# XiaRho/CMDA

Measured on AMD Instinct MI355X. Metric: training images/sec (512x512 image+event, MiT-B5), higher is better.
Workload: dtype bf16

## Files before the change

cmda_amd/csrc/attention.hip:

```cpp
#include "attention_common.h"

namespace {

struct AttnParams {
  const bf16_t* q;
  const bf16_t* kv;
  bf16_t* o;
  int B, N, Nk, heads, C;
  float scale;
  int q_per_block;
};

static inline int fwd_queries_per_block(int B, int N, int heads, bool full = false) {
  return (long)((N + 127) / 128) * heads * B < (full ? 512 : 1024) ? 64 : 128;
}

template <int MAXK, bool FULL = false>
__global__ __launch_bounds__(256, MAXK <= 256 ? 2 : 1) void attn_fwd_kernel(AttnParams p) {
  constexpr int NT = MAXK / 16;
  const int Nk = FULL ? MAXK : p.Nk;
  __shared__ __attribute__((aligned(1024))) bf16_t sK[MAXK * kHD];
  __shared__ __attribute__((aligned(1024))) bf16_t sV[MAXK * kHD];
  const int tid = threadIdx.x, lane = tid & 63, wid = tid >> 6, g = lane >> 4, l15 = lane & 15;
  const unsigned nqb = (unsigned)((p.N + p.q_per_block - 1) / p.q_per_block);
  const unsigned lb = xcd_logical_block(), bh = lb / nqb;
  const long qblk = lb - bh * nqb;
  const int h = (int)(bh % (unsigned)p.heads), b = (int)(bh / (unsigned)p.heads);
  const bf16_t* kbase = p.kv + (long)b * Nk * 2 * p.C + h * kHD;
  load_kv_tile<MAXK>(kbase, 2 * p.C, Nk, sK, wid, lane, 4);
  load_kv_tile<MAXK>(kbase + p.C, 2 * p.C, Nk, sV, wid, lane, 4);
  __syncthreads();
  const int nt = (Nk + 15) >> 4;
  const bf16_t* qb = p.q + (long)b * p.N * p.C + h * kHD;
  bf16_t* ob = p.o + (long)b * p.N * p.C + h * kHD;
  for (int pass = 0; pass < p.q_per_block / 64; ++pass) {
    const long q0 = qblk * p.q_per_block + pass * 64 + wid * 16;
    if (q0 >= p.N) break;
    u16x8 qf[2];
    load_qfrag(qb, q0, p.N, p.C, g, l15, qf);
    f32x4 pr[NT];
    float inv = 1.f;
    if constexpr (FULL) inv = scores_exp_full<NT>(sK, qf, p.scale, g, l15, pr);
    else scores_softmax<NT>(sK, qf, nt, Nk, p.scale, g, l15, pr);
    f32x4 oacc[4];
#pragma unroll
    for (int dt = 0; dt < 4; ++dt) oacc[dt] = f32x4{0.f, 0.f, 0.f, 0.f};
#pragma unroll
    for (int u = 0; u < NT / 2; ++u) {
      if (FULL || 2 * u < nt) {
        const u16x8 pb = pack_pair(pr[2 * u], pr[2 * u + 1]);
#pragma unroll
        for (int dt = 0; dt < 4; ++dt)
          oacc[dt] = mfma_bf16_16x16x32(frag_cols(sV, 32 * u + 4 * g, 32 * u + 16 + 4 * g, dt, l15), pb, oacc[dt]);
      }
    }
    if (q0 + l15 < p.N) {
#pragma unroll
      for (int dt = 0; dt < 4; ++dt) {
        if constexpr (FULL) oacc[dt] *= inv;
        const float v[4] = {oacc[dt][0], oacc[dt][1], oacc[dt][2], oacc[dt][3]};
        st4(ob + (q0 + l15) * p.C + 16 * dt + 4 * g, v);
      }
    }
  }
}

struct AttnBwdParams {
  const bf16_t* q;
  const bf16_t* kv;
  const bf16_t* d_o;
  bf16_t* dq;
  float* dkv32;
  bf16_t* dkv16;
  float* stats;
  int B, N, Nk, heads, C, q_per_block;
  float scale;
  int fwd_q_per_block;
  int spans;
};

template <bool FULL = false>
__global__ __launch_bounds__(256, 2) void attn_bwd_dq_kernel(AttnBwdParams p) {
  __shared__ __attribute__((aligned(1024))) bf16_t sK[kMaxK * kHD];
  __shared__ __attribute__((aligned(1024))) bf16_t sV[kMaxK * kHD];
  const int Nk = FULL ? kMaxK : p.Nk;
  const int tid = threadIdx.x, lane = tid & 63, wid = tid >> 6, g = lane >> 4, l15 = lane & 15;
  const unsigned nqb = (unsigned)((p.N + p.fwd_q_per_block - 1) / p.fwd_q_per_block);
  const unsigned lb = xcd_logical_block(), bh = lb / nqb;
  const long qblk = lb - bh * nqb;
  const int h = (int)(bh % (unsigned)p.heads), b = (int)(bh / (unsigned)p.heads);
  const bf16_t* kbase = p.kv + (long)b * Nk * 2 * p.C + h * kHD;
  load_kv_tile(kbase, 2 * p.C, Nk, sK, wid, lane, 4);
  load_kv_tile(kbase + p.C, 2 * p.C, Nk, sV, wid, lane, 4);
  __syncthreads();
  const int nt = (Nk + 15) >> 4;
  const long rowb = (long)b * p.N;
  const bf16_t* qb = p.q + rowb * p.C + h * kHD;
  const bf16_t* dob = p.d_o + rowb * p.C + h * kHD;
  bf16_t* dqb = p.dq + rowb * p.C + h * kHD;
  float* st = p.stats + ((long)b * p.heads + h) * p.N * 2;
  for (int pass = 0; pass < p.fwd_q_per_block / 64; ++pass) {
    const long q0 = qblk * p.fwd_q_per_block + pass * 64 + wid * 16;
    if (q0 >= p.N) break;
    u16x8 qf[2], dof[2];
    load_qfrag(qb, q0, p.N, p.C, g, l15, qf);
    load_qfrag(dob, q0, p.N, p.C, g, l15, dof);
    f32x4 pr[kNT], dp[kNT];
    float lse, inv = 1.f;
    if constexpr (FULL) inv = scores_exp_full(sK, qf, p.scale, g, l15, pr, &lse);
    else scores_softmax(sK, qf, nt, Nk, p.scale, g, l15, pr, &lse);
    float dsum = 0.f;
#pragma unroll
    for (int t = 0; t < kNT; ++t) {
      dp[t] = f32x4{0.f, 0.f, 0.f, 0.f};
      if (FULL || t < nt) {
#pragma unroll
        for (int kk = 0; kk < 2; ++kk) dp[t] = mfma_bf16_16x16x32(frag_rows(sV, 16 * t, kk, g, l15), dof[kk], dp[t]);
      }
#pragma unroll
      for (int r = 0; r < 4; ++r) dsum += pr[t][r] * dp[t][r];
    }
    dsum = col_sum(dsum);
    if constexpr (FULL) dsum *= inv;
#pragma unroll
    for (int t = 0; t < kNT; ++t)
#pragma unroll
      for (int r = 0; r < 4; ++r) {
        if constexpr (FULL) dp[t][r] = pr[t][r] * (dp[t][r] - dsum);
        else dp[t][r] = p.scale * pr[t][r] * (dp[t][r] - dsum);
      }
    f32x4 dqacc[4];
#pragma unroll
    for (int dt = 0; dt < 4; ++dt) dqacc[dt] = f32x4{0.f, 0.f, 0.f, 0.f};
#pragma unroll
    for (int u = 0; u < kNT / 2; ++u) {
      if (FULL || 2 * u < nt) {
        const u16x8 db = pack_pair(dp[2 * u], dp[2 * u + 1]);
#pragma unroll
        for (int dt = 0; dt < 4; ++dt)
          dqacc[dt] = mfma_bf16_16x16x32(frag_cols(sK, 32 * u + 4 * g, 32 * u + 16 + 4 * g, dt, l15), db, dqacc[dt]);
      }
    }
    if (q0 + l15 < p.N) {
#pragma unroll
      for (int dt = 0; dt < 4; ++dt) {
        if constexpr (FULL) dqacc[dt] *= p.scale * inv;
        const float v[4] = {dqacc[dt][0], dqacc[dt][1], dqacc[dt][2], dqacc[dt][3]};
        st4(dqb + (q0 + l15) * p.C + 16 * dt + 4 * g, v);
      }
      if (g == 0) {
        st[(q0 + l15) * 2 + 0] = lse;
        st[(q0 + l15) * 2 + 1] = dsum;
      }
    }
  }
}

constexpr int kRedPitch = 68;

template <int NW>
__global__ __launch_bounds__(64 * NW, NW == 4 ? 2 : 1) void attn_bwd_dkv_kernel(AttnBwdParams p) {
  __shared__ __attribute__((aligned(1024))) bf16_t sK[kKS * kHD];
  __shared__ __attribute__((aligned(1024))) bf16_t sV[kKS * kHD];
  constexpr int kStageBytes = NW * 2 * 32 * kHD * 2;
  constexpr int kRedBytes = 2 * kKS * kRedPitch * 4;
  __shared__ __attribute__((aligned(1024))) char sbuf[kStageBytes > kRedBytes ? kStageBytes : kRedBytes];
  const int tid = threadIdx.x, lane = tid & 63, wid = tid >> 6, g = lane >> 4, l15 = lane & 15;
  const unsigned lb = xcd_logical_block();
  const int ks = (int)(lb & 3);
  const unsigned span = (lb >> 2) % (unsigned)p.spans, bh = (lb >> 2) / (unsigned)p.spans;
  const int h = (int)(bh % (unsigned)p.heads), b = (int)(bh / (unsigned)p.heads);
  const int key0 = ks * kKS;
  if (key0 >= p.Nk) return;
  const int nkeys = min(kKS, p.Nk - key0);
  const bf16_t* kbase = p.kv + ((long)b * p.Nk + key0) * 2 * p.C + h * kHD;
  for (int i = wid; i < kKS / 8; i += NW) {
    const int row = 8 * i + (lane >> 3);
    const int chunk = (lane & 7) ^ (row & 7);
    const void* zero = static_cast<const void*>(g_attn_zero16);
    const bf16_t* src = kbase + (long)row * 2 * p.C + chunk * 8;
    glds16(row < nkeys ? static_cast<const void*>(src) : zero, reinterpret_cast<char*>(sK) + i * 1024);
    glds16(row < nkeys ? static_cast<const void*>(src + p.C) : zero, reinterpret_cast<char*>(sV) + i * 1024);
  }
  __syncthreads();
  const long rowb = (long)b * p.N;
  const bf16_t* qb = p.q + rowb * p.C + h * kHD;
  const bf16_t* dob = p.d_o + rowb * p.C + h * kHD;
  const float* st = p.stats + ((long)b * p.heads + h) * p.N * 2;
  bf16_t* sQw = reinterpret_cast<bf16_t*>(sbuf) + wid * 2 * 32 * kHD;
  bf16_t* sDOw = sQw + 32 * kHD;

  f32x4 dvacc[4][4], dkacc[4][4];
#pragma unroll
  for (int dt = 0; dt < 4; ++dt)
#pragma unroll
    for (int kt = 0; kt < 4; ++kt) dvacc[dt][kt] = dkacc[dt][kt] = f32x4{0.f, 0.f, 0.f, 0.f};

  const long qbeg = (long)span * p.q_per_block;
  const long qend = min((long)p.N, qbeg + p.q_per_block);
  for (long q32 = qbeg + 32 * wid; q32 < qend; q32 += 32 * NW) {
#pragma unroll
    for (int i = 0; i < 4; ++i) {
      const int row = 8 * i + (lane >> 3);
      const int chunk = (lane & 7) ^ (row & 7);
      const bool ok = q32 + row < p.N;
      const void* zero = static_cast<const void*>(g_attn_zero16);
      glds16(ok ? static_cast<const void*>(qb + (q32 + row) * p.C + chunk * 8) : zero, reinterpret_cast<char*>(sQw) + i * 1024);
      glds16(ok ? static_cast<const void*>(dob + (q32 + row) * p.C + chunk * 8) : zero, reinterpret_cast<char*>(sDOw) + i * 1024);
    }
    float lse[2][4], dd[2][4];
#pragma unroll
    for (int qt = 0; qt < 2; ++qt)
#pragma unroll
      for (int r = 0; r < 4; ++r) {
        const long qi = q32 + 16 * qt + 4 * g + r;
        const bool ok = qi < p.N;
        lse[qt][r] = ok ? st[qi * 2] : INFINITY;
        dd[qt][r] = ok ? st[qi * 2 + 1] : 0.f;
      }
    dma_wait<0>();
    f32x4 pr[2][4], ds[2][4];
#pragma unroll
    for (int qt = 0; qt < 2; ++qt) {
      u16x8 fq[2], fdo[2];
#pragma unroll
      for (int kk = 0; kk < 2; ++kk) {
        fq[kk] = frag_rows(sQw, 16 * qt, kk, g, l15);
        fdo[kk] = frag_rows(sDOw, 16 * qt, kk, g, l15);
      }
#pragma unroll
      for (int kt = 0; kt < 4; ++kt) {
        f32x4 s = f32x4{0.f, 0.f, 0.f, 0.f}, d = f32x4{0.f, 0.f, 0.f, 0.f};
#pragma unroll
        for (int kk = 0; kk < 2; ++kk) {
          s = mfma_bf16_16x16x32(fq[kk], frag_rows(sK, 16 * kt, kk, g, l15), s);
          d = mfma_bf16_16x16x32(fdo[kk], frag_rows(sV, 16 * kt, kk, g, l15), d);
        }
        const bool live = 16 * kt + l15 < nkeys;
#pragma unroll
        for (int r = 0; r < 4; ++r) {
          const float pv = live ? __expf(s[r] * p.scale - lse[qt][r]) : 0.f;
          pr[qt][kt][r] = pv;
          ds[qt][kt][r] = p.scale * pv * (d[r] - dd[qt][r]);
        }
      }
    }
#pragma unroll
    for (int dt = 0; dt < 4; ++dt) {
      const u16x8 fdoT = frag_cols(sDOw, 4 * g, 16 + 4 * g, dt, l15);
      const u16x8 fqT = frag_cols(sQw, 4 * g, 16 + 4 * g, dt, l15);
#pragma unroll
      for (int kt = 0; kt < 4; ++kt) {
        dvacc[dt][kt] = mfma_bf16_16x16x32(fdoT, pack_pair(pr[0][kt], pr[1][kt]), dvacc[dt][kt]);
        dkacc[dt][kt] = mfma_bf16_16x16x32(fqT, pack_pair(ds[0][kt], ds[1][kt]), dkacc[dt][kt]);
      }
    }
  }
  __syncthreads();
  float* red = reinterpret_cast<float*>(sbuf);
  for (int w = 0; w < NW; ++w) {
    if (wid == w) {
#pragma unroll
      for (int dt = 0; dt < 4; ++dt)
#pragma unroll
        for (int kt = 0; kt < 4; ++kt) {
          float* rk = red + (16 * kt + l15) * kRedPitch + 16 * dt + 4 * g;
          float* rv = rk + kKS * kRedPitch;
#pragma unroll
          for (int r = 0; r < 4; ++r) {
            rk[r] = (w ? rk[r] : 0.f) + dkacc[dt][kt][r];
            rv[r] = (w ? rv[r] : 0.f) + dvacc[dt][kt][r];
          }
        }
    }
    __syncthreads();
  }
  if (p.dkv16) {
    bf16_t* ob = p.dkv16 + ((long)b * p.Nk + key0) * 2 * p.C + h * kHD;
    for (int e = tid; e < kKS * kHD; e += 64 * NW) {
      const int kl = e >> 6, d = e & 63;
      if (kl < nkeys) {
        stf(ob + (long)kl * 2 * p.C + d, red[kl * kRedPitch + d]);
        stf(ob + (long)kl * 2 * p.C + p.C + d, red[(kKS + kl) * kRedPitch + d]);
      }
    }
    return;
  }
  float* ob = p.dkv32 + ((long)b * p.Nk + key0) * 2 * p.C + h * kHD;
  for (int e = tid; e < kKS * kHD; e += 64 * NW) {
    const int kl = e >> 6, d = e & 63;
    if (kl < nkeys) {
      atomicAdd(ob + (long)kl * 2 * p.C + d, red[kl * kRedPitch + d]);
      atomicAdd(ob + (long)kl * 2 * p.C + p.C + d, red[(kKS + kl) * kRedPitch + d]);
    }
  }
}


struct AttnX3Params {
  const float* q;
  const bf16_t* kvh;
  const bf16_t* kvl;
  float* o;
  int B, N, Nk, heads, C;
  float scale;
  int q_per_block;
};

static __device__ __forceinline__ void split4(const float (&x)[4], u16x4& hi, u16x4& lo) {
#pragma unroll
  for (int e = 0; e < 4; ++e) {
    const bf16_t h = f2bf(x[e]);
    hi[e] = h;
    lo[e] = f2bf(x[e] - bf2f(h));
  }
}

#ifndef CMDA_EMU
static __device__ __forceinline__ void wave_lds_sync() { asm volatile("s_waitcnt lgkmcnt(0)" ::: "memory"); }
#else
static inline void wave_lds_sync() { emu::wave_barrier(); }
#endif

static __device__ __forceinline__ void load_split_tile(const float* __restrict__ src, long ld, int nvalid, int rows, bf16_t* hi, bf16_t* lo,
                                                       int t, int nthr) {
  for (int i = t; i < rows * 16; i += nthr) {
    const int row = i >> 4, c4 = i & 15;
    float x[4] = {0.f, 0.f, 0.f, 0.f};
    if (row < nvalid) ld4(src + (long)row * ld + 4 * c4, x);
    u16x4 h, l;
    split4(x, h, l);
    const int off = row * kHD + ((((c4 >> 1) ^ (row & 7))) << 3) + ((c4 & 1) << 2);
    *reinterpret_cast<u16x4*>(hi + off) = h;
    *reinterpret_cast<u16x4*>(lo + off) = l;
  }
}

static __device__ __forceinline__ void load_qfrag_x3(const float* __restrict__ base, long row0, long nrows, int ld, int g, int l15,
                                                     u16x8 (&fh)[2], u16x8 (&fl)[2]) {
  long row = row0 + l15;
  if (row >= nrows) row = nrows - 1;
#pragma unroll
  for (int kk = 0; kk < 2; ++kk) {
    float a[4], b[4];
    ld4(base + row * ld + 32 * kk + 8 * g, a);
    ld4(base + row * ld + 32 * kk + 8 * g + 4, b);
    u16x4 ah, al, bh, bl;
    split4(a, ah, al);
    split4(b, bh, bl);
    fh[kk] = u16x8{ah[0], ah[1], ah[2], ah[3], bh[0], bh[1], bh[2], bh[3]};
    fl[kk] = u16x8{al[0], al[1], al[2], al[3], bl[0], bl[1], bl[2], bl[3]};
  }
}

static __device__ __forceinline__ f32x4 mfma_x3(u16x8 ah, u16x8 al, u16x8 bh, u16x8 bl, f32x4 c) {
  c = mfma_bf16_16x16x32(al, bh, c);
  c = mfma_bf16_16x16x32(ah, bl, c);
  return mfma_bf16_16x16x32(ah, bh, c);
}

static __device__ __forceinline__ void pack_pair_x3(const f32x4& a, const f32x4& b, u16x8& hi, u16x8& lo) {
#pragma unroll
  for (int r = 0; r < 4; ++r) {
    const bf16_t ha = f2bf(a[r]), hb = f2bf(b[r]);
    hi[r] = ha; hi[4 + r] = hb;
    lo[r] = f2bf(a[r] - bf2f(ha)); lo[4 + r] = f2bf(b[r] - bf2f(hb));
  }
}

static __device__ __forceinline__ void scores_softmax_x3(const bf16_t* sKh, const bf16_t* sKl, const u16x8 (&qh)[2], const u16x8 (&ql)[2],
                                                         int nt, int Nk, float scale, int g, int l15, f32x4 (&p)[kNT], float* lse_out = nullptr) {
#pragma unroll
  for (int t = 0; t < kNT; ++t) {
    p[t] = f32x4{0.f, 0.f, 0.f, 0.f};
    if (t < nt) {
#pragma unroll
      for (int kk = 0; kk < 2; ++kk)
// ... 242 lines not shown
        fdh[kk] = frag_rows(sDh, 16 * qt, kk, g, l15);
        fdl[kk] = frag_rows(sDl, 16 * qt, kk, g, l15);
      }
#pragma unroll
      for (int kt = 0; kt < 4; ++kt) {
        f32x4 s = f32x4{0.f, 0.f, 0.f, 0.f}, d = f32x4{0.f, 0.f, 0.f, 0.f};
#pragma unroll
        for (int kk = 0; kk < 2; ++kk) {
          s = mfma_x3(fqh[kk], fql[kk], frag_rows(sKh, 16 * kt, kk, g, l15), frag_rows(sKl, 16 * kt, kk, g, l15), s);
          d = mfma_x3(fdh[kk], fdl[kk], frag_rows(sVh, 16 * kt, kk, g, l15), frag_rows(sVl, 16 * kt, kk, g, l15), d);
        }
        const bool live = 16 * kt + l15 < nkeys;
#pragma unroll
        for (int r = 0; r < 4; ++r) {
          const float pv = live ? __expf(s[r] * p.scale - lse[qt][r]) : 0.f;
          pr[qt][kt][r] = pv;
          ds[qt][kt][r] = p.scale * pv * (d[r] - dd[qt][r]);
        }
      }
    }
#pragma unroll
    for (int dt = 0; dt < 4; ++dt) {
      const u16x8 fdoTh = frag_cols(sDh, 4 * g, 16 + 4 * g, dt, l15), fdoTl = frag_cols(sDl, 4 * g, 16 + 4 * g, dt, l15);
      const u16x8 fqTh = frag_cols(sQh, 4 * g, 16 + 4 * g, dt, l15), fqTl = frag_cols(sQl, 4 * g, 16 + 4 * g, dt, l15);
#pragma unroll
      for (int kt = 0; kt < 4; ++kt) {
        u16x8 ph, pl, dh, dl;
        pack_pair_x3(pr[0][kt], pr[1][kt], ph, pl);
        pack_pair_x3(ds[0][kt], ds[1][kt], dh, dl);
        dvacc[dt][kt] = mfma_x3(fdoTh, fdoTl, ph, pl, dvacc[dt][kt]);
        dkacc[dt][kt] = mfma_x3(fqTh, fqTl, dh, dl, dkacc[dt][kt]);
      }
    }
  }
  __syncthreads();
  float* red = reinterpret_cast<float*>(sbuf);
  for (int w = 0; w < NW; ++w) {
    if (wid == w) {
#pragma unroll
      for (int dt = 0; dt < 4; ++dt)
#pragma unroll
        for (int kt = 0; kt < 4; ++kt) {
          float* rk = red + (16 * kt + l15) * kRedPitch + 16 * dt + 4 * g;
          float* rv = rk + kKS * kRedPitch;
#pragma unroll
          for (int r = 0; r < 4; ++r) {
            rk[r] = (w ? rk[r] : 0.f) + dkacc[dt][kt][r];
            rv[r] = (w ? rv[r] : 0.f) + dvacc[dt][kt][r];
          }
        }
    }
    __syncthreads();
  }
  if (p.dkv_out) {
    float* ob = p.dkv_out + ((long)b * p.Nk + key0) * 2 * p.C + h * kHD;
    for (int e = tid; e < kKS * kHD; e += 64 * NW) {
      const int kl = e >> 6, d = e & 63;
      if (kl < nkeys) {
        ob[(long)kl * 2 * p.C + d] = red[kl * kRedPitch + d];
        ob[(long)kl * 2 * p.C + p.C + d] = red[(kKS + kl) * kRedPitch + d];
      }
    }
    return;
  }
  float* ob = p.dkv32 + ((long)b * p.Nk + key0) * 2 * p.C + h * kHD;
  for (int e = tid; e < kKS * kHD; e += 64 * NW) {
    const int kl = e >> 6, d = e & 63;
    if (kl < nkeys) {
      atomicAdd(ob + (long)kl * 2 * p.C + d, red[kl * kRedPitch + d]);
      atomicAdd(ob + (long)kl * 2 * p.C + p.C + d, red[(kKS + kl) * kRedPitch + d]);
    }
  }
}

}

static inline bool head_dim_ok(int heads, int C) {
  const int hd = C / heads;
  return C == heads * hd && hd % kHD == 0 && hd >= kHD && hd <= 1024;
}

static inline bool attn_full_keys(int Nk, float scale) { return Nk == kMaxK && scale > 0.f; }

extern "C" int cmda_attention_fwd(const void* q, const void* kv, void* o, int B, int N, int Nk, int heads, int C,
                                  float scale, int dtype, void* stream) {
  if (B <= 0 || N <= 0) return CMDA_OK;
  if (dtype != CMDA_BF16) return CMDA_ERR_DTYPE;
  if (heads <= 0 || Nk <= 0 || Nk > kMaxKFwd || !head_dim_ok(heads, C)) return CMDA_ERR_UNSUPPORTED;
  if (heads > 65535 || B > 65535) return CMDA_ERR_SHAPE;
  if (C != heads * kHD) return attn_wide_fwd(q, kv, o, B, N, Nk, heads, C, scale, stream);
  const bool full = attn_full_keys(Nk, scale);
  const int qpb = fwd_queries_per_block(B, N, heads, full);
  AttnParams p{(const bf16_t*)q, (const bf16_t*)kv, (bf16_t*)o, B, N, Nk, heads, C, scale, qpb};
  const long nblk = (long)((N + qpb - 1) / qpb) * heads * B;
  if (nblk > 0x7fffffffL) return CMDA_ERR_SHAPE;
  dim3 grid((unsigned)nblk);
  if (full) CMDA_LAUNCH((attn_fwd_kernel<kMaxK, true>), grid, dim3(256), 0, stream, p);
  else if (Nk <= kMaxK) CMDA_LAUNCH(attn_fwd_kernel<kMaxK>, grid, dim3(256), 0, stream, p);
  else CMDA_LAUNCH(attn_fwd_kernel<kMaxKFwd>, grid, dim3(256), 0, stream, p);
  CMDA_CHECK_LAUNCH();
}

extern "C" int64_t cmda_attention_bwd_ws_floats(int B, int N, int heads) { return (int64_t)B * N * heads * 2; }

extern "C" int cmda_attention_bwd_direct(int B, int N, int Nk, int heads) {
  (void)B; (void)heads;
  return N <= 1024 && Nk <= kMaxK ? 1 : 0;
}

extern "C" int cmda_attention_bwd(const void* q, const void* kv, const void* d_o, void* dq, float* dkv32, void* dkv16,
                                  float* stats, int B, int N, int Nk, int heads, int C, float scale, int dtype, void* stream) {
  if (B <= 0 || N <= 0) return CMDA_OK;
  if (dtype != CMDA_BF16) return CMDA_ERR_DTYPE;
  if (heads <= 0 || Nk <= 0 || Nk > kMaxK || !head_dim_ok(heads, C)) return CMDA_ERR_UNSUPPORTED;
  if (heads * 4 > 65535 || B > 65535) return CMDA_ERR_SHAPE;
  if (C != heads * kHD) {
    if (dkv32 == nullptr) return CMDA_ERR_SHAPE;
    return attn_wide_bwd(q, kv, d_o, dq, dkv32, stats, B, N, Nk, heads, C, scale, stream);
  }
  const bool direct = cmda_attention_bwd_direct(B, N, Nk, heads) != 0 && dkv16 != nullptr;
  if (!direct && dkv32 == nullptr) return CMDA_ERR_SHAPE;
  const bool full = attn_full_keys(Nk, scale);
  const int fqpb = fwd_queries_per_block(B, N, heads, full);
  AttnBwdParams p{(const bf16_t*)q, (const bf16_t*)kv, (const bf16_t*)d_o, (bf16_t*)dq, dkv32, direct ? (bf16_t*)dkv16 : nullptr, stats,
                  B, N, Nk, heads, C, 0, scale, fqpb};
  const long nblk1 = (long)((N + fqpb - 1) / fqpb) * heads * B;
  if (nblk1 > 0x7fffffffL) return CMDA_ERR_SHAPE;
  dim3 g1((unsigned)nblk1);
  if (full) CMDA_LAUNCH(attn_bwd_dq_kernel<true>, g1, dim3(256), 0, stream, p);
  else CMDA_LAUNCH(attn_bwd_dq_kernel<false>, g1, dim3(256), 0, stream, p);
  const long slices = (long)B * heads * ((Nk + kKS - 1) / kKS);
  long spans = direct ? 1 : std::max<long>(1, 512 / slices);
  long qpb = ((N + spans - 1) / spans + 127) / 128 * 128;
  spans = (N + qpb - 1) / qpb;
  p.q_per_block = (int)qpb;
  p.spans = (int)spans;
  dim3 g2((unsigned)(spans * heads * 4 * B));
  if (direct && N > 512) CMDA_LAUNCH(attn_bwd_dkv_kernel<8>, g2, dim3(512), 0, stream, p);
  else CMDA_LAUNCH(attn_bwd_dkv_kernel<4>, g2, dim3(256), 0, stream, p);
  CMDA_CHECK_LAUNCH();
}

extern "C" int cmda_attention_fwd_x3(const float* q, const void* kv_hi, const void* kv_lo, float* o, int B, int N, int Nk, int heads, int C,
                                     float scale, void* stream) {
  if (B <= 0 || N <= 0) return CMDA_OK;
  if (heads <= 0 || C != heads * kHD || Nk <= 0 || Nk > kMaxK || (C & 3)) return CMDA_ERR_UNSUPPORTED;
  if (heads > 65535 || B > 65535) return CMDA_ERR_SHAPE;
  const int qpb = (long)((N + 127) / 128) * heads * B < 256 ? 64 : 128;
  AttnX3Params p{q, (const bf16_t*)kv_hi, (const bf16_t*)kv_lo, o, B, N, Nk, heads, C, scale, qpb};
  const long nblk = (long)((N + qpb - 1) / qpb) * heads * B;
  if (nblk > 0x7fffffffL) return CMDA_ERR_SHAPE;
  CMDA_LAUNCH(attn_fwd_x3_kernel, dim3((unsigned)nblk), dim3(256), 0, stream, p);
  CMDA_CHECK_LAUNCH();
}

extern "C" int cmda_attention_bwd_x3(const float* q, const void* kv_hi, const void* kv_lo, const float* d_o, float* dq, float* dkv32,
                                     float* dkv_direct, float* stats, int B, int N, int Nk, int heads, int C, float scale, void* stream) {
  if (B <= 0 || N <= 0) return CMDA_OK;
  if (heads <= 0 || C != heads * kHD || Nk <= 0 || Nk > kMaxK || (C & 3)) return CMDA_ERR_UNSUPPORTED;
  if (heads * 4 > 65535 || B > 65535) return CMDA_ERR_SHAPE;
  const bool direct = cmda_attention_bwd_direct(B, N, Nk, heads) != 0 && dkv_direct != nullptr;
  if (!direct && dkv32 == nullptr) return CMDA_ERR_SHAPE;
  const int fq = (long)((N + 127) / 128) * heads * B < 256 ? 64 : 128;
  AttnBwdX3Params p{q, (const bf16_t*)kv_hi, (const bf16_t*)kv_lo, d_o, dq, dkv32, direct ? dkv_direct : nullptr, stats,
                    B, N, Nk, heads, C, 0, scale, fq, 1};
  const long nb1 = (long)((N + fq - 1) / fq) * heads * B;
  if (nb1 > 0x7fffffffL) return CMDA_ERR_SHAPE;
  CMDA_LAUNCH(attn_bwd_dq_x3_kernel, dim3((unsigned)nb1), dim3(256), 0, stream, p);
  const long slices = (long)B * heads * ((Nk + kKS - 1) / kKS);
  long spans = direct ? 1 : std::max<long>(1, 256 / slices);
  long qpb = ((N + spans - 1) / spans + 127) / 128 * 128;
  spans = (N + qpb - 1) / qpb;
  p.q_per_block = (int)qpb;
  p.spans = (int)spans;
  CMDA_LAUNCH(attn_bwd_dkv_x3_kernel, dim3((unsigned)(spans * heads * 4 * B)), dim3(256), 0, stream, p);
  CMDA_CHECK_LAUNCH();
}
```

cmda_amd/ops.py:

```python
import ctypes
import os

import numpy as np
import torch

from . import _lib as L
from . import deferred as D
from ._lib import BF16, F32, GemmParams, View, c_f32, c_i32, c_i64, call, check_dev, dtype_tag, ptr, stream_of

_ESIZE = {torch.float32: 4, torch.bfloat16: 2}


def _chunk(t):
    return 16 // _ESIZE[t.dtype]


def plain_view(t, rows, cols, ld=None, batch_stride=0, offset=0, batch2_stride=0):
    ld = cols if ld is None else ld
    es = _ESIZE[t.dtype]
    ch = 16 // es
    base = t.data_ptr() + offset * es
    vec_ok = int(base % 16 == 0 and ld % ch == 0 and batch_stride % ch == 0 and batch2_stride % ch == 0)
    v = View(ptr=base, ld=ld, R=rows, Cc=cols, batch_stride=batch_stride, batch2_stride=batch2_stride, conv=0,
             vec_ok=vec_ok,
# ... 415 lines not shown
    call('cmda_adamw_step', ptr(p), ptr(g), ptr(m), ptr(v), ptr(p_bf16), c_i64(p.numel()), c_f32(lr), c_f32(beta1),
         c_f32(beta2), c_f32(eps), c_f32(wd), c_i32(step), stream_of(p))


def class_mix(src, tgt, src_label, classes, channels_last=False):
    check_dev(src, tgt, src_label, classes)
    out = torch.empty_like(src)
    B = src.shape[0]
    HW = src_label.shape[-2] * src_label.shape[-1]
    Cch = src.numel() // (B * HW)
    call('cmda_class_mix', ptr(src), ptr(tgt), ptr(out), ptr(src_label), ptr(classes), c_i32(classes.shape[1]), c_i32(B),
         c_i32(HW), c_i32(Cch), c_i32(int(channels_last)), dtype_tag(src), stream_of(src))
    return out


def class_mix_label(src, tgt, src_label, classes):
    check_dev(src, tgt, src_label, classes)
    out = torch.empty_like(src)
    B = src.shape[0]
    call('cmda_class_mix_label', ptr(src), ptr(tgt), ptr(out), ptr(src_label), ptr(classes), c_i32(classes.shape[1]),
         c_i32(B), c_i32(src.numel() // B), stream_of(src))
    return out


def softmax_fwd_(s, rows, L, alpha):
    check_dev(s)
    call('cmda_softmax_fwd', ptr(s), c_i64(rows), c_i32(L), c_f32(alpha), dtype_tag(s), stream_of(s))
    return s


def softmax_bwd_(p, dp, rows, L, alpha):
    check_dev(p, dp)
    call('cmda_softmax_bwd', ptr(p), ptr(dp), c_i64(rows), c_i32(L), c_f32(alpha), dtype_tag(p), stream_of(p))
    return dp


ATTN_WIDE_TABLE = {128: (True, True), 256: (True, False), 320: (False, False), 512: (False, False), 640: (False, False),
                   1024: (False, False)}


def attention_fused_ok(q, Nk, heads, C, need_grad=True, x3=False):
    if x3 and q.dtype == torch.float32:
        return C == heads * 64 and 0 < Nk <= 256 and not ATTN_X3_OFF
    if q.dtype != torch.bfloat16 or heads <= 0 or C % heads or not 0 < Nk <= (256 if need_grad else 320):
        return False
    hd = C // heads
    if hd == 64:
        return True
    mode = os.environ.get('CMDA_ATTN_WIDE', '1')
    if hd % 64 or not 64 < hd <= 1024 or mode == '0':
        return False
    return mode == '2' or ATTN_WIDE_TABLE.get(hd, (False, False))[1 if need_grad else 0]


ATTN_X3_OFF = os.environ.get('CMDA_ATTN_X3', '1') == '0'


def _kv_split(kv):
    pair = getattr(kv, '_cmda_split', None)
    if pair is None or pair[2] != kv._version:
        hi, lo = split_bf16(kv)
        pair = kv._cmda_split = (hi, lo, kv._version)
    return pair[0], pair[1]


def attention_fused_fwd(q, kv, B, N, Nk, heads, C, scale):
    check_dev(q, kv)
    o = torch.empty(B * N, C, dtype=q.dtype, device=q.device)
    if q.dtype == torch.float32:
        hi, lo = _kv_split(kv)
        _attn_profile(4.0 * B * N * Nk * C, lambda: call('cmda_attention_fwd_x3', ptr(q), ptr(hi), ptr(lo), ptr(o), c_i32(B), c_i32(N),
                                                         c_i32(Nk), c_i32(heads), c_i32(C), c_f32(scale), stream_of(q)))
        return o
    _attn_profile(4.0 * B * N * Nk * C, lambda: call('cmda_attention_fwd', ptr(q), ptr(kv), ptr(o), c_i32(B), c_i32(N), c_i32(Nk),
                                                     c_i32(heads), c_i32(C), c_f32(scale), dtype_tag(q), stream_of(q)))
    return o


def attention_fwd_queries_per_block(B, N, heads, Nk=256, scale=0.125):
    full = int(Nk) == 256 and scale > 0
    return 64 if -(-int(N) // 128) * int(heads) * int(B) < (512 if full else 1024) else 128


def attention_bwd_direct(B, N, Nk, heads):
    return bool(L.lib().cmda_attention_bwd_direct(int(B), int(N), int(Nk), int(heads)))


def attention_fused_bwd(q, kv, do, dkv32, B, N, Nk, heads, C, scale, dkv16=None):
    check_dev(q, kv, do, dkv32, dkv16)
    dq = torch.empty(B * N, C, dtype=q.dtype, device=q.device)
    stats = torch.empty(B * N * heads * 2, dtype=torch.float32, device=q.device)
    if q.dtype == torch.float32:
        hi, lo = _kv_split(kv)
        _attn_profile(10.0 * B * N * Nk * C, lambda: call('cmda_attention_bwd_x3', ptr(q), ptr(hi), ptr(lo), ptr(do), ptr(dq), ptr(dkv32),
                                                          ptr(dkv16), ptr(stats), c_i32(B), c_i32(N), c_i32(Nk), c_i32(heads), c_i32(C),
                                                          c_f32(scale), stream_of(q)))
        return dq
    _attn_profile(10.0 * B * N * Nk * C, lambda: call('cmda_attention_bwd', ptr(q), ptr(kv), ptr(do), ptr(dq), ptr(dkv32), ptr(dkv16),
                                                      ptr(stats), c_i32(B), c_i32(N), c_i32(Nk), c_i32(heads), c_i32(C), c_f32(scale),
                                                      dtype_tag(q), stream_of(q)))
    return dq


def dwconv_fwd(x, w, bias, B, H, W, C, dil=1, act=None, colstats=None):
    check_dev(x, w, bias)
    y = torch.empty_like(x)
    if colstats is not None:
        assert act is None and dil >= 2
        check_dev(colstats[0])
        call('cmda_dwconv3x3_fwd_stats', ptr(x), ptr(w), ptr(bias), ptr(y), c_i32(B), c_i32(H), c_i32(W), c_i32(C), c_i32(dil),
             ptr(colstats[0]), c_i32(colstats[1]), dtype_tag(x), stream_of(x))
        return y
    call('cmda_dwconv3x3_fwd', ptr(x), ptr(w), ptr(bias), ptr(y), c_i32(B), c_i32(H), c_i32(W), c_i32(C), c_i32(dil),
         c_i32(ACT[act]), dtype_tag(x), stream_of(x))
    return y


def dwconv_gelu_bwd_prep(x, w, bias, da, B, H, W, C, dil=1):
    check_dev(x, w, bias, da)
    dz = torch.empty_like(x)
    call('cmda_dwconv3x3_gelu_bwd_prep', ptr(x), ptr(w), ptr(bias), ptr(da), ptr(dz), c_i32(B), c_i32(H), c_i32(W),
         c_i32(C), c_i32(dil), dtype_tag(x), stream_of(x))
    return dz


def dwconv_gelu_bwd_fused(x, w, bias, da, dw, dbias, B, H, W, C, dil=1):
    check_dev(x, w, bias, da, dw, dbias)
    dz = torch.empty_like(x)
    call('cmda_dwconv3x3_gelu_bwd_fused', ptr(x), ptr(w), ptr(bias), ptr(da), ptr(dz), ptr(dw), ptr(dbias), c_i32(B), c_i32(H),
         c_i32(W), c_i32(C), c_i32(dil), dtype_tag(x), stream_of(x))
    return dz


def dwconv_bwd_data(dy, w, B, H, W, C, dil=1, out=None, accumulate=False):
    check_dev(dy, w, out)
    dx = torch.empty_like(dy) if out is None else out
    call('cmda_dwconv3x3_bwd_data', ptr(dy), ptr(w), ptr(dx), c_i32(B), c_i32(H), c_i32(W), c_i32(C), c_i32(dil),
         c_i32(int(accumulate)), dtype_tag(dy), stream_of(dy))
    return dx


def dwconv_bwd_weight(dz, x, dw, dbias, B, H, W, C, dil=1):
    check_dev(dz, x, dw, dbias)
    call('cmda_dwconv3x3_bwd_weight', ptr(dz), ptr(x), ptr(dw), ptr(dbias), c_i32(B), c_i32(H), c_i32(W), c_i32(C),
         c_i32(dil), dtype_tag(x), stream_of(x))


def bilinear_fwd(x, y, B, IH, IW, OH, OW, C, ldy=None, coff=0):
    check_dev(x, y)
    call('cmda_bilinear_fwd', ptr(x), ptr(y), c_i32(B), c_i32(IH), c_i32(IW), c_i32(OH), c_i32(OW), c_i32(C),
         c_i32(C if ldy is None else ldy), c_i32(coff), dtype_tag(x), stream_of(x))
    return y


def bilinear_bwd(dy, dx, B, IH, IW, OH, OW, C, ldy=None, coff=0):
    check_dev(dy, dx)
    call('cmda_bilinear_bwd', ptr(dy), ptr(dx), c_i32(B), c_i32(IH), c_i32(IW), c_i32(OH), c_i32(OW), c_i32(C),
         c_i32(C if ldy is None else ldy), c_i32(coff), dtype_tag(dy), stream_of(dy))
    return dx


BN_FUSED_STATS = os.environ.get('CMDA_BN_FUSED_STATS', '1') != '0'
def bn_stats_ws(device, groups, C):
    if not BN_FUSED_STATS:
        return None
    need = groups * int(L.lib().cmda_bn_ws_floats(C))
# ... 615 lines not shown
```

Baseline: 40.36.

## Restructure attention dK/dV backward kernel: register-resident K/V slices with double-buffered Q/dO

The dK/dV backward kernel now has each wave own one 16-key tile, holding its K/V fragments and dK/dV accumulators in registers instead of reading shared-memory K/V tiles. Q/dO tiles are double-buffered so the next tile's global-to-LDS load and stats load overlap compute. The full-key case switches to exp2 with a prescaled log-sum-exp. Key-slice size and query-group count are picked per shape, and the serial cross-wave reduction becomes a single park-and-sum. This adds many template instantiations, an environment override, and a different grid split whose occupancy tradeoffs are hard to predict.

```diff
diff --git a/cmda_amd/csrc/attention.hip b/cmda_amd/csrc/attention.hip
--- a/cmda_amd/csrc/attention.hip
+++ b/cmda_amd/csrc/attention.hip
@@ -1,4 +1,6 @@
 #include "attention_common.h"
+#include <cstdio>
+#include <cstdlib>
 
 namespace {
 
@@ -157,142 +159,180 @@
 }
 
 constexpr int kRedPitch = 68;
-
-template <int NW>
-__global__ __launch_bounds__(64 * NW, NW == 4 ? 2 : 1) void attn_bwd_dkv_kernel(AttnBwdParams p) {
-  __shared__ __attribute__((aligned(1024))) bf16_t sK[kKS * kHD];
-  __shared__ __attribute__((aligned(1024))) bf16_t sV[kKS * kHD];
-  constexpr int kStageBytes = NW * 2 * 32 * kHD * 2;
-  constexpr int kRedBytes = 2 * kKS * kRedPitch * 4;
+constexpr int kParkPitch = 132;
+
+template <int KS, int QG, bool FULL>
+__global__ __launch_bounds__(4 * KS * QG) void attn_bwd_dkv_kernel(AttnBwdParams p) {
+  constexpr int KT = KS / 16, NW = KT * QG, TQ = 32 * QG;
+  constexpr int kTile = TQ * kHD;
+  constexpr int kStageBytes = 2 * 2 * kTile * 2;
+  constexpr int kRedBytes = NW * 16 * kParkPitch * 4;
   __shared__ __attribute__((aligned(1024))) char sbuf[kStageBytes > kRedBytes ? kStageBytes : kRedBytes];
+  const int Nk = FULL ? kMaxK : p.Nk;
   const int tid = threadIdx.x, lane = tid & 63, wid = tid >> 6, g = lane >> 4, l15 = lane & 15;
+  const int kt = wid % KT, qg = wid / KT;
+  const unsigned nsl = (unsigned)((Nk + KS - 1) / KS);
   const unsigned lb = xcd_logical_block();
-  const int ks = (int)(lb & 3);
-  const unsigned span = (lb >> 2) % (unsigned)p.spans, bh = (lb >> 2) / (unsigned)p.spans;
+  const unsigned ks = lb % nsl, rest = lb / nsl;
+  const unsigned span = rest % (unsigned)p.spans, bh = rest / (unsigned)p.spans;
   const int h = (int)(bh % (unsigned)p.heads), b = (int)(bh / (unsigned)p.heads);
-  const int key0 = ks * kKS;
-  if (key0 >= p.Nk) return;
-  const int nkeys = min(kKS, p.Nk - key0);
-  const bf16_t* kbase = p.kv + ((long)b * p.Nk + key0) * 2 * p.C + h * kHD;
-  for (int i = wid; i < kKS / 8; i += NW) {
-    const int row = 8 * i + (lane >> 3);
-    const int chunk = (lane & 7) ^ (row & 7);
-    const void* zero = static_cast<const void*>(g_attn_zero16);
-    const bf16_t* src = kbase + (long)row * 2 * p.C + chunk * 8;
-    glds16(row < nkeys ? static_cast<const void*>(src) : zero, reinterpret_cast<char*>(sK) + i * 1024);
-    glds16(row < nkeys ? static_cast<const void*>(src + p.C) : zero, reinterpret_cast<char*>(sV) + i * 1024);
-  }
-  __syncthreads();
+  const int key = (int)ks * KS + 16 * kt + l15;
+  const bool live = FULL || key < Nk;
+  const long krow = ((long)b * Nk + (live ? key : Nk - 1)) * 2 * p.C + h * kHD;
+  u16x8 fk[2], fv[2];
+#pragma unroll
+  for (int kk = 0; kk < 2; ++kk) {
+    fk[kk] = *reinterpret_cast<const u16x8*>(p.kv + krow + 32 * kk + 8 * g);
+    fv[kk] = *reinterpret_cast<const u16x8*>(p.kv + krow + p.C + 32 * kk + 8 * g);
+  }
   const long rowb = (long)b * p.N;
   const bf16_t* qb = p.q + rowb * p.C + h * kHD;
   const bf16_t* dob = p.d_o + rowb * p.C + h * kHD;
   const float* st = p.stats + ((long)b * p.heads + h) * p.N * 2;
-  bf16_t* sQw = reinterpret_cast<bf16_t*>(sbuf) + wid * 2 * 32 * kHD;
-  bf16_t* sDOw = sQw + 32 * kHD;
-
-  f32x4 dvacc[4][4], dkacc[4][4];
-#pragma unroll
-  for (int dt = 0; dt < 4; ++dt)
-#pragma unroll
-    for (int kt = 0; kt < 4; ++kt) dvacc[dt][kt] = dkacc[dt][kt] = f32x4{0.f, 0.f, 0.f, 0.f};
+  bf16_t* stage = reinterpret_cast<bf16_t*>(sbuf);
+
+  auto issue = [&](long q0, int buf) {
+    char* sQ = reinterpret_cast<char*>(stage + buf * 2 * kTile);
+    char* sDO = sQ + kTile * 2;
+#pragma unroll
+    for (int j = 0; j < 4 / KT; ++j) {
+      const int i = wid + j * NW;
+      const int row = 8 * i + (lane >> 3);
+      const int chunk = (lane & 7) ^ (row & 7);
+      const bool ok = q0 + row < p.N;
+      const void* zero = static_cast<const void*>(g_attn_zero16);
+      glds16(ok ? static_cast<const void*>(qb + (q0 + row) * p.C + chunk * 8) : zero, sQ + i * 1024);
+      glds16(ok ? static_cast<const void*>(dob + (q0 + row) * p.C + chunk * 8) : zero, sDO + i * 1024);
+    }
+  };
+  auto load_stats = [&](long q0, float2 (&sv)[2][4]) {
+#pragma unroll
+    for (int qt = 0; qt < 2; ++qt)
+#pragma unroll
+      for (int r = 0; r < 4; ++r) {
+        const long qi = q0 + 32 * qg + 16 * qt + 4 * g + r;
+        sv[qt][r] = *reinterpret_cast<const float2*>(st + min(qi, (long)p.N - 1) * 2);
+      }
+  };
+
+  f32x4 dvacc[4], dkacc[4];
+#pragma unroll
+  for (int dt = 0; dt < 4; ++dt) dvacc[dt] = dkacc[dt] = f32x4{0.f, 0.f, 0.f, 0.f};
 
   const long qbeg = (long)span * p.q_per_block;
   const long qend = min((long)p.N, qbeg + p.q_per_block);
-  for (long q32 = qbeg + 32 * wid; q32 < qend; q32 += 32 * NW) {
-#pragma unroll
-    for (int i = 0; i < 4; ++i) {
-      const int row = 8 * i + (lane >> 3);
-      const int chunk = (lane & 7) ^ (row & 7);
-      const bool ok = q32 + row < p.N;
-      const void* zero = static_cast<const void*>(g_attn_zero16);
-      glds16(ok ? static_cast<const void*>(qb + (q32 + row) * p.C + chunk * 8) : zero, reinterpret_cast<char*>(sQw) + i * 1024);
-      glds16(ok ? static_cast<const void*>(dob + (q32 + row) * p.C + chunk * 8) : zero, reinterpret_cast<char*>(sDOw) + i * 1024);
-    }
+  const int ntiles = (int)((qend - qbeg + TQ - 1) / TQ);
+  const float c = p.scale * 1.44269504088896340736f;
+  float2 sv[2][4];
+  issue(qbeg, 0);
+  load_stats(qbeg, sv);
+  for (int i = 0; i < ntiles; ++i) {
+    dma_wait<0>();
+    __syncthreads();
+    const long q0 = qbeg + (long)i * TQ;
     float lse[2][4], dd[2][4];
 #pragma unroll
     for (int qt = 0; qt < 2; ++qt)
 #pragma unroll
       for (int r = 0; r < 4; ++r) {
-        const long qi = q32 + 16 * qt + 4 * g + r;
-        const bool ok = qi < p.N;
-        lse[qt][r] = ok ? st[qi * 2] : INFINITY;
-        dd[qt][r] = ok ? st[qi * 2 + 1] : 0.f;
-      }
-    dma_wait<0>();
-    f32x4 pr[2][4], ds[2][4];
+        const bool ok = q0 + 32 * qg + 16 * qt + 4 * g + r < p.N;
+        const float l = ok ? sv[qt][r].x : INFINITY;
+        lse[qt][r] = FULL ? -1.44269504088896340736f * l : l;
+        dd[qt][r] = ok ? sv[qt][r].y : 0.f;
+      }
+    const bool have = q0 + 32 * qg < qend;
+    const bf16_t* sQ = stage + (i & 1) * 2 * kTile + 32 * qg * kHD;
+    const bf16_t* sDO = sQ + kTile;
+    u16x8 fdoT[4], fqT[4];
+    if (have) {
+#pragma unroll
+      for (int dt = 0; dt < 4; ++dt) {
+        fdoT[dt] = frag_cols(sDO, 4 * g, 16 + 4 * g, dt, l15);
+        fqT[dt] = frag_cols(sQ, 4 * g, 16 + 4 * g, dt, l15);
+      }
+    }
+    if (i + 1 < ntiles) {
+      issue(q0 + TQ, (i + 1) & 1);
+      load_stats(q0 + TQ, sv);
+    }
+    if (!have) continue;
+    f32x4 pr[2], ds[2];
 #pragma unroll
     for (int qt = 0; qt < 2; ++qt) {
-      u16x8 fq[2], fdo[2];
+      f32x4 s = f32x4{0.f, 0.f, 0.f, 0.f}, d = f32x4{0.f, 0.f, 0.f, 0.f};
 #pragma unroll
       for (int kk = 0; kk < 2; ++kk) {
-        fq[kk] = frag_rows(sQw, 16 * qt, kk, g, l15);
-        fdo[kk] = frag_rows(sDOw, 16 * qt, kk, g, l15);
-      }
-#pragma unroll
-      for (int kt = 0; kt < 4; ++kt) {
-        f32x4 s = f32x4{0.f, 0.f, 0.f, 0.f}, d = f32x4{0.f, 0.f, 0.f, 0.f};
-#pragma unroll
-        for (int kk = 0; kk < 2; ++kk) {
-          s = mfma_bf16_16x16x32(fq[kk], frag_rows(sK, 16 * kt, kk, g, l15), s);
-          d = mfma_bf16_16x16x32(fdo[kk], frag_rows(sV, 16 * kt, kk, g, l15), d);
+        s = mfma_bf16_16x16x32(frag_rows(sQ, 16 * qt, kk, g, l15), fk[kk], s);
+        d = mfma_bf16_16x16x32(frag_rows(sDO, 16 * qt, kk, g, l15), fv[kk], d);
+      }
+#pragma unroll
+      for (int r = 0; r < 4; ++r) {
+        if constexpr (FULL) {
+          const float pv = fast_exp2(fmaf(s[r], c, lse[qt][r]));
+          pr[qt][r] = pv;
+          ds[qt][r] = pv * (d[r] - dd[qt][r]);
+        } else {
+          const float pv = live ? __expf(s[r] * p.scale - lse[qt][r]) : 0.f;
+          pr[qt][r] = pv;
+          ds[qt][r] = p.scale * pv * (d[r] - dd[qt][r]);
         }
-        const bool live = 16 * kt + l15 < nkeys;
-#pragma unroll
-        for (int r = 0; r < 4; ++r) {
-          const float pv = live ? __expf(s[r] * p.scale - lse[qt][r]) : 0.f;
-          pr[qt][kt][r] = pv;
-          ds[qt][kt][r] = p.scale * pv * (d[r] - dd[qt][r]);
-        }
-      }
-    }
+      }
+    }
+    const u16x8 pb = pack_pair(pr[0], pr[1]), db = pack_pair(ds[0], ds[1]);
 #pragma unroll
     for (int dt = 0; dt < 4; ++dt) {
-      const u16x8 fdoT = frag_cols(sDOw, 4 * g, 16 + 4 * g, dt, l15);
-      const u16x8 fqT = frag_cols(sQw, 4 * g, 16 + 4 * g, dt, l15);
-#pragma unroll
-      for (int kt = 0; kt < 4; ++kt) {
-        dvacc[dt][kt] = mfma_bf16_16x16x32(fdoT, pack_pair(pr[0][kt], pr[1][kt]), dvacc[dt][kt]);
-        dkacc[dt][kt] = mfma_bf16_16x16x32(fqT, pack_pair(ds[0][kt], ds[1][kt]), dkacc[dt][kt]);
-      }
-    }
+      dvacc[dt] = mfma_bf16_16x16x32(fdoT[dt], pb, dvacc[dt]);
+      dkacc[dt] = mfma_bf16_16x16x32(fqT[dt], db, dkacc[dt]);
+    }
+  }
+  if constexpr (FULL) {
+#pragma unroll
+    for (int dt = 0; dt < 4; ++dt) dkacc[dt] *= p.scale;
+  }
+  const long orow = ((long)b * Nk + key) * 2 * p.C + h * kHD;
+  auto col = [&](int a) { return (a < 4 ? kHD : 0) + 16 * (a & 3) + 4 * g; };
+  auto store16 = [&](int a, const f32x4& v) {
+    if (!live) return;
+    const int c = col(a);
+    const float f[4] = {v[0], v[1], v[2], v[3]};
+    st4(p.dkv16 + orow + (c < kHD ? c : p.C + c - kHD), f);
+  };
+  if (QG == 1 && p.dkv16) {
+#pragma unroll
+    for (int dt = 0; dt < 4; ++dt) {
+      store16(dt, dvacc[dt]);
+      store16(4 + dt, dkacc[dt]);
+    }
+    return;
   }
   __syncthreads();
   float* red = reinterpret_cast<float*>(sbuf);
-  for (int w = 0; w < NW; ++w) {
-    if (wid == w) {
-#pragma unroll
-      for (int dt = 0; dt < 4; ++dt)
-#pragma unroll
-        for (int kt = 0; kt < 4; ++kt) {
-          float* rk = red + (16 * kt + l15) * kRedPitch + 16 * dt + 4 * g;
-          float* rv = rk + kKS * kRedPitch;
-#pragma unroll
-          for (int r = 0; r < 4; ++r) {
-            rk[r] = (w ? rk[r] : 0.f) + dkacc[dt][kt][r];
-            rv[r] = (w ? rv[r] : 0.f) + dvacc[dt][kt][r];
-          }
-        }
-    }
-    __syncthreads();
-  }
+#pragma unroll
+  for (int dt = 0; dt < 4; ++dt) {
+    *reinterpret_cast<f32x4*>(red + (wid * 16 + l15) * kParkPitch + col(dt)) = dvacc[dt];
+    *reinterpret_cast<f32x4*>(red + (wid * 16 + l15) * kParkPitch + col(4 + dt)) = dkacc[dt];
+  }
+  __syncthreads();
   if (p.dkv16) {
-    bf16_t* ob = p.dkv16 + ((long)b * p.Nk + key0) * 2 * p.C + h * kHD;
-    for (int e = tid; e < kKS * kHD; e += 64 * NW) {
-      const int kl = e >> 6, d = e & 63;
-      if (kl < nkeys) {
-        stf(ob + (long)kl * 2 * p.C + d, red[kl * kRedPitch + d]);
-        stf(ob + (long)kl * 2 * p.C + p.C + d, red[(kKS + kl) * kRedPitch + d]);
-      }
+#pragma unroll
+    for (int j = 0; j < 8 / QG; ++j) {
+      const int a = qg * (8 / QG) + j;
+      f32x4 sum = *reinterpret_cast<const f32x4*>(red + (kt * 16 + l15) * kParkPitch + col(a));
+#pragma unroll
+      for (int g2 = 1; g2 < QG; ++g2) sum += *reinterpret_cast<const f32x4*>(red + ((g2 * KT + kt) * 16 + l15) * kParkPitch + col(a));
+      store16(a, sum);
     }
     return;
   }
-  float* ob = p.dkv32 + ((long)b * p.Nk + key0) * 2 * p.C + h * kHD;
-  for (int e = tid; e < kKS * kHD; e += 64 * NW) {
-    const int kl = e >> 6, d = e & 63;
-    if (kl < nkeys) {
-      atomicAdd(ob + (long)kl * 2 * p.C + d, red[kl * kRedPitch + d]);
-      atomicAdd(ob + (long)kl * 2 * p.C + p.C + d, red[(kKS + kl) * kRedPitch + d]);
-    }
+#pragma unroll
+  for (int j = 0; j < 32 / QG; ++j) {
+    const int row = qg * (32 / QG) + j;
+    const int kl = row >> 1, kg = (int)ks * KS + 16 * kt + kl;
+    if (!FULL && kg >= Nk) continue;
+    float sum = red[(kt * 16 + kl) * kParkPitch + (row & 1) * kHD + lane];
+#pragma unroll
+    for (int g2 = 1; g2 < QG; ++g2) sum += red[((g2 * KT + kt) * 16 + kl) * kParkPitch + (row & 1) * kHD + lane];
+    atomicAdd(p.dkv32 + ((long)b * Nk + kg) * 2 * p.C + h * kHD + (row & 1) * p.C + lane, sum);
   }
 }
 
@@ -701,6 +741,57 @@
 
 static inline bool attn_full_keys(int Nk, float scale) { return Nk == kMaxK && scale > 0.f; }
 
+struct DkvConfig { int ks, qg; long span_q; };
+
+constexpr long kDkvBlocks = 256;
+static inline DkvConfig dkv_default_config(int B, int N, int heads, bool direct) {
+  const long bh = (long)B * heads;
+  if (!direct) return DkvConfig{32, 4, 0};
+  const int ks = bh * (kMaxK / 16) <= kDkvBlocks ? 16 : bh * (kMaxK / 32) <= kDkvBlocks ? 32 : 64;
+  const int groups = (N + 31) / 32;
+  return DkvConfig{ks, groups >= 4 && ks < 64 ? 4 : groups >= 2 ? 2 : 1, 0};
+}
+
+static inline bool dkv_forced_config(DkvConfig* c) {
+  const char* e = getenv("CMDA_ATTN_DKV");
+  if (!e || !*e) return false;
+  int ks = 0, qg = 0;
+  long sq = 0;
+  const int n = sscanf(e, "%d,%d,%ld", &ks, &qg, &sq);
+  *c = DkvConfig{n >= 2 ? ks : -1, n >= 2 ? qg : -1, n >= 3 && sq > 0 ? sq : 0};
+  return true;
+}
+
+template <bool FULL>
+static int launch_dkv_inst(const AttnBwdParams& p, int ks, int qg, dim3 grid, void* stream) {
+#define CMDA_DKV_CASE(KS, QG)                                                                                          \
+  if (ks == KS && qg == QG) {                                                                                          \
+    CMDA_LAUNCH((attn_bwd_dkv_kernel<KS, QG, FULL>), grid, dim3(4 * KS * QG), 0, stream, p);                            \
+    CMDA_CHECK_LAUNCH();                                                                                               \
+  }
+  CMDA_DKV_CASE(64, 1) CMDA_DKV_CASE(64, 2)
+  CMDA_DKV_CASE(32, 1) CMDA_DKV_CASE(32, 2) CMDA_DKV_CASE(32, 4)
+  CMDA_DKV_CASE(16, 1) CMDA_DKV_CASE(16, 2) CMDA_DKV_CASE(16, 4)
+#undef CMDA_DKV_CASE
+  return CMDA_ERR_UNSUPPORTED;
+}
+
+static int launch_dkv(AttnBwdParams p, bool direct, bool full, void* stream) {
+  DkvConfig c;
+  if (!dkv_forced_config(&c)) c = dkv_default_config(p.B, p.N, p.heads, direct);
+  if (c.ks <= 0 || c.qg <= 0) return CMDA_ERR_UNSUPPORTED;
+  const long slices = (long)p.B * p.heads * ((p.Nk + c.ks - 1) / c.ks);
+  long spans = 1;
+  if (!direct) spans = c.span_q ? (p.N + c.span_q - 1) / c.span_q : std::max<long>(1, kDkvBlocks / slices);
+  const long qpb = ((p.N + spans - 1) / spans + 127) / 128 * 128;
+  spans = (p.N + qpb - 1) / qpb;
+  if (spans * slices > 0x7fffffffL) return CMDA_ERR_SHAPE;
+  p.q_per_block = (int)qpb;
+  p.spans = (int)spans;
+  const dim3 grid((unsigned)(spans * slices));
+  return full ? launch_dkv_inst<true>(p, c.ks, c.qg, grid, stream) : launch_dkv_inst<false>(p, c.ks, c.qg, grid, stream);
+}
+
 extern "C" int cmda_attention_fwd(const void* q, const void* kv, void* o, int B, int N, int Nk, int heads, int C,
                                   float scale, int dtype, void* stream) {
   if (B <= 0 || N <= 0) return CMDA_OK;
@@ -748,16 +839,7 @@
   dim3 g1((unsigned)nblk1);
   if (full) CMDA_LAUNCH(attn_bwd_dq_kernel<true>, g1, dim3(256), 0, stream, p);
   else CMDA_LAUNCH(attn_bwd_dq_kernel<false>, g1, dim3(256), 0, stream, p);
-  const long slices = (long)B * heads * ((Nk + kKS - 1) / kKS);
-  long spans = direct ? 1 : std::max<long>(1, 512 / slices);
-  long qpb = ((N + spans - 1) / spans + 127) / 128 * 128;
-  spans = (N + qpb - 1) / qpb;
-  p.q_per_block = (int)qpb;
-  p.spans = (int)spans;
-  dim3 g2((unsigned)(spans * heads * 4 * B));
-  if (direct && N > 512) CMDA_LAUNCH(attn_bwd_dkv_kernel<8>, g2, dim3(512), 0, stream, p);
-  else CMDA_LAUNCH(attn_bwd_dkv_kernel<4>, g2, dim3(256), 0, stream, p);
-  CMDA_CHECK_LAUNCH();
+  return launch_dkv(p, direct, full, stream);
 }
 
 extern "C" int cmda_attention_fwd_x3(const float* q, const void* kv_hi, const void* kv_lo, float* o, int B, int N, int Nk, int heads, int C,
diff --git a/cmda_amd/ops.py b/cmda_amd/ops.py
--- a/cmda_amd/ops.py
+++ b/cmda_amd/ops.py
@@ -521,6 +521,19 @@
     return 64 if -(-int(N) // 128) * int(heads) * int(B) < (512 if full else 1024) else 128
 
 
+def attention_dkv_config(B, N, heads, Nk=256):
+    B, N, heads, Nk = int(B), int(N), int(heads), int(Nk)
+    bh = B * heads
+    if N <= 1024 and Nk <= 256:
+        ks = 16 if bh * 16 <= 256 else 32 if bh * 8 <= 256 else 64
+        groups = -(-N // 32)
+        return ks, 4 if groups >= 4 and ks < 64 else 2 if groups >= 2 else 1, 1
+    ks, qg = 32, 4
+    spans = max(1, 256 // (bh * -(-Nk // ks)))
+    qpb = -(-(-(-N // spans)) // 128) * 128
+    return ks, qg, -(-N // qpb)
+
+
 def attention_bwd_direct(B, N, Nk, heads):
     return bool(L.lib().cmda_attention_bwd_direct(int(B), int(N), int(Nk), int(heads)))
 
```

Result: no change. 40.07 (-0.7%).
